# YukunXia/SuperPoint-Stereo-Visual-Odometry

Measured on AMD Instinct MI355X. Metric: stereo frames/sec (1241x376 KITTI), higher is better.
Workload: dtype f32

## Files before the change

superpoint-stereo-visual-odometry_amd/csrc/conv_wino4.hip.h:

```cpp
#pragma once
#include <hip/hip_runtime.h>
#include <stdint.h>
#include <type_traits>
#include <vector>
#include "conv_mfma.hip.h"

#ifndef WINO4_LEAD
#define WINO4_LEAD 6
#endif
#ifndef WINO4_PRIO
#define WINO4_PRIO 1
#endif
#ifndef WINO4_H1_STEPS
#define WINO4_H1_STEPS 6
#endif
#ifndef WINO4_H1_START
#define WINO4_H1_START 3
#endif
#ifndef WINO4_H1_STRIDE
#define WINO4_H1_STRIDE 5
#endif
#ifndef WINO4_H2_START
#define WINO4_H2_START 4
#endif
#ifndef WINO4_H2_STRIDE
#define WINO4_H2_STRIDE 8
#endif
#ifndef WINO4_ABL
#define WINO4_ABL 0
#endif

#ifndef SPVO_STATIC_BANDS
#define SPVO_STATIC_BANDS 1
#endif

namespace spvo {

template <int TB>
struct Wino4TileT {
  static constexpr int CK = 4, TH = 8 * TB, TW = 32, LW = TW + 8, LH = TH + 2, NT = 16 * TB, NTH = 256 * TB;
  static constexpr int IN_FLOATS = CK * LH * LW;
  static constexpr int U_FLOATS = 36 * CK * CO_TILE;
  static constexpr int V_FLOATS = 10 * TB * 64 * 4;
  static constexpr int RAW_OFF = 0, U_OFF = 2 * IN_FLOATS, V_OFF = U_OFF + 2 * U_FLOATS;
  static constexpr int LDS_BYTES = (V_OFF + 2 * V_FLOATS) * 4 + 16;
};
using Wino4Tile = Wino4TileT<2>;

inline std::vector<float> pack_conv_weights_wino4(const float *w, const float *bias, int cout, int cin) {
  constexpr int CK = Wino4Tile::CK;
  const int co_tiles = (cout + CO_TILE - 1) / CO_TILE, nch = cin / CK;
  std::vector<float> out((size_t)co_tiles * nch * Wino4Tile::U_FLOATS + (size_t)co_tiles * CO_TILE, 0.f);
  static const double G[6][3] = {{0.25, 0, 0}, {-1.0 / 6, -1.0 / 6, -1.0 / 6}, {-1.0 / 6, 1.0 / 6, -1.0 / 6},
                                 {1.0 / 24, 1.0 / 12, 1.0 / 6}, {1.0 / 24, -1.0 / 12, 1.0 / 6}, {0, 0, 1}};
  for (int ct = 0; ct < co_tiles; ++ct)
    for (int o = 0; o < CO_TILE; ++o) {
      const int co = ct * CO_TILE + o;
      if (co >= cout) continue;
      out[(size_t)co_tiles * nch * Wino4Tile::U_FLOATS + co] = bias[co];
      for (int ci = 0; ci < cin; ++ci) {
        const float *g = w + ((size_t)co * cin + ci) * 9;
        double t[6][3];
        for (int a = 0; a < 6; ++a)
          for (int k = 0; k < 3; ++k) t[a][k] = G[a][0] * g[0 * 3 + k] + G[a][1] * g[1 * 3 + k] + G[a][2] * g[2 * 3 + k];
        float *slab = out.data() + ((size_t)ct * nch + ci / CK) * Wino4Tile::U_FLOATS;
        const int lane = 16 * (ci % CK) + (o & 15), cq = o >> 4;
        for (int a = 0; a < 6; ++a)
          for (int b = 0; b < 6; ++b) {
            const int pos = 18 * (b / 3) + 3 * a + b % 3;
            slab[(((pos >> 2) * 4 + cq) * 64 + lane) * 4 + (pos & 3)] = (float)(t[a][0] * G[b][0] + t[a][1] * G[b][1] + t[a][2] * G[b][2]);
          }
      }
    }
  return out;
}

__device__ __forceinline__ void wino4_in6(const float x0, const float x1, const float x2, const float x3, const float x4, const float x5, float (&o)[6]) {
  const float e = fmaf(-4.f, x2, x4), od = fmaf(-4.f, x1, x3), e2 = x4 - x2, o2 = x3 - x1;
  o[0] = fmaf(4.f, x0, fmaf(-5.f, x2, x4));
  o[1] = e + od;
  o[2] = e - od;
  o[3] = fmaf(2.f, o2, e2);
  o[4] = fmaf(-2.f, o2, e2);
  o[5] = fmaf(4.f, x1, fmaf(-5.f, x3, x5));
}
__device__ __forceinline__ void wino4_out4(const float m0, const float m1, const float m2, const float m3, const float m4, const float m5, float (&y)[4]) {
  const float a = m1 + m2, b = m1 - m2, c = m3 + m4, d = m3 - m4;
  y[0] = (m0 + a) + c;
  y[1] = fmaf(2.f, d, b);
  y[2] = fmaf(4.f, c, a);
  y[3] = fmaf(8.f, d, b) + m5;
}

typedef float wino4_f32x2 __attribute__((ext_vector_type(2)));
__device__ __forceinline__ void wino4_out4(const wino4_f32x2 m0, const wino4_f32x2 m1, const wino4_f32x2 m2, const wino4_f32x2 m3, const wino4_f32x2 m4,
                                           const wino4_f32x2 m5, wino4_f32x2 (&y)[4]) {
  const wino4_f32x2 a = m1 + m2, b = m1 - m2, c = m3 + m4, d = m3 - m4;
  y[0] = (m0 + a) + c;
  y[1] = __builtin_elementwise_fma(wino4_f32x2{2.f, 2.f}, d, b);
  y[2] = __builtin_elementwise_fma(wino4_f32x2{4.f, 4.f}, c, a);
  y[3] = __builtin_elementwise_fma(wino4_f32x2{8.f, 8.f}, d, b) + m5;
}

template <bool POOL, bool RELU, int TAG = 0, int TB = 2>
__global__ __launch_bounds__(256 * TB, TB) void conv_wino4_kernel(const ConvArgs a) {
  using T = Wino4TileT<TB>;
  constexpr int CK = T::CK, LW = T::LW, LH = T::LH, LW4 = LW / 4, NTH = T::NTH;
  constexpr int IN_V4 = T::IN_FLOATS / 4;
  constexpr int U_V4 = T::U_FLOATS / 4;
  constexpr int NIT_U = (U_V4 + NTH - 1) / NTH;
  typedef float f32x2 __attribute__((ext_vector_type(2)));
  typedef float f32x4v __attribute__((ext_vector_type(4)));

  extern __shared__ __attribute__((aligned(16))) float smem[];

  const int tid = threadIdx.x;
  const int lane = tid & 63;
  const int c16 = lane & 15, g4 = lane >> 4;
  const int wave = __builtin_amdgcn_readfirstlane(tid >> 6);
  const int cq = wave & 3, tb = wave >> 2;
  const size_t in_plane = (size_t)a.in_hp * a.in_wp;
  const size_t out_plane = (size_t)a.out_hp * a.out_wp;
  const int n_tiles = a.tiles_x * a.tiles_y * a.co_tiles * a.batch;

  struct TileRef { const float *in_base, *w_base; int x0, y0, ct, img; };
  auto decode = [&](int id) {
    TileRef t;
    const int tx = id % a.tiles_x;
    id /= a.tiles_x;
    const int ty = id % a.tiles_y;
    id /= a.tiles_y;
    t.ct = id % a.co_tiles;
    t.img = id / a.co_tiles;
    t.x0 = tx * T::TW;
    t.y0 = ty * T::TH;
    t.in_base = a.in + ((size_t)t.img * a.in_ctot + a.in_coff) * in_plane + (size_t)(t.y0 + PADY - 1) * a.in_wp + (t.x0 + PADX - 4);
    t.w_base = a.wpack + (size_t)t.ct * a.n_chunks * T::U_FLOATS;
    return t;
  };

  auto raw_piece_off = [&](int idx) {
    idx = min(idx, IN_V4 - 1);
    const int ci = idx / (LH * LW4);
    const int rem = idx - ci * (LH * LW4);
    const int r = rem / LW4;
    const int q = rem - r * LW4;
    return 4u * (unsigned)(ci * (int)in_plane + r * a.in_wp + q * 4);
  };
  constexpr int R0 = NTH - 256;
  const unsigned roff0 = raw_piece_off(tid), roff1 = raw_piece_off(NTH + (tid - R0));
  const bool raw2 = tid >= R0 && NTH + (tid - R0) < IN_V4;
  auto issue_raw = [&](const TileRef &t, int chunk, float *buf) {
    const char *inb = reinterpret_cast<const char *>(t.in_base + (size_t)chunk * CK * in_plane);
    glds16(reinterpret_cast<const float *>(inb + roff0), buf + (wave * 64) * 4);
    if (raw2) glds16(reinterpret_cast<const float *>(inb + roff1), buf + (NTH + (wave - R0 / 64) * 64) * 4);
  };
  const unsigned uoff = 16u * (unsigned)tid;
  auto issue_u = [&](const TileRef &t, int chunk, float *buf) {
    const char *wb = reinterpret_cast<const char *>(t.w_base + (size_t)chunk * T::U_FLOATS);
#pragma unroll
    for (int it = 0; it < NIT_U; ++it)
      if (it < NIT_U - 1 || tid < U_V4 - (NIT_U - 1) * NTH) glds16(reinterpret_cast<const float *>(wb + (uoff + 16u * NTH * it)), buf + (it * NTH + wave * 64) * 4);
  };

  const int x_ci = TB == 2 ? (wave & 3) : 2 * (wave & 1) + ((lane >> 4) & 1), x_tile = TB == 2 ? (lane & 31) : (lane & 15), x_h = lane >> 5;
  const int x_trow = x_tile >> 3, x_tcol = x_tile & 7;
  const int raw_off = x_ci * (LH * LW) + (4 * x_trow + 3 * x_h) * LW + 4 * x_tcol + 3;
  const int v_off = x_h * (1280 * TB) + (x_tile >> 4) * 256 + (16 * x_ci + (x_tile & 15)) * 4;
  float xr[3][6];
  f32x4v xa[3];
  float xs0[3], xs1[3];
  auto xf_step = [&](const float *raw, float *vb, int st) {
    if (st < 3) {
      const float *d = raw + raw_off + st * LW;
      xs0[st] = d[0];
      xa[st] = *reinterpret_cast<const f32x4v *>(d + 1);
      xs1[st] = d[5];
    } else if (st < 6) {
      const int r = st - 3;
      wino4_in6(xs0[r], xa[r][0], xa[r][1], xa[r][2], xa[r][3], xs1[r], xr[r]);
    } else if (st == 6) {
#pragma unroll
      for (int r = 0; r < 3; ++r)
#pragma unroll
        for (int c = 0; c < 3; ++c) {
          typedef unsigned u32x2s __attribute__((ext_vector_type(2)));
          const u32x2s sw = __builtin_amdgcn_permlane32_swap(__float_as_uint(xr[r][c]), __float_as_uint(xr[r][c + 3]), false, false);
          xr[r][c] = __uint_as_float(sw[0]);
          xr[r][c + 3] = __uint_as_float(sw[1]);
        }
    } else {
      const int c = st - 7;
      float o[6];
      wino4_in6(xr[0][c], xr[1][c], xr[2][c], xr[0][c + 3], xr[1][c + 3], xr[2][c + 3], o);
#pragma unroll
      for (int i = 0; i < 6; ++i) vb[v_off + ((3 * i + c) >> 2) * (256 * TB) + ((3 * i + c) & 3)] = o[i];
    }
  };

  const int a_lane = cq * 64 + lane;
  const int b_lane = tb * 64 + lane;

  const int band = blockIdx.x & 7;
  auto wgs_before = [&](int b) { return min(b, (int)gridDim.x & 7) + b * ((int)gridDim.x >> 3); };
  auto band_lo = [&](int b) { return (int)((long)n_tiles * wgs_before(b) / (int)gridDim.x); };
  auto band_hi = [&](int b) { return band_lo(b + 1); };
  auto band_wgs = [&](int b) { return wgs_before(b + 1) - wgs_before(b); };
  auto steal = [&]() {
    for (int k = 1; k < 8; ++k) {
      const int b = (band + k) & 7;
      if (band_lo(b) + band_wgs(b) >= band_hi(b)) continue;
      const int v = band_lo(b) + band_wgs(b) + atomicAdd(a.sched + b, 1);
      if (v < band_hi(b)) return v;
    }
    return n_tiles;
  };
  auto all_done = [&]() {
    if (a.sched && tid == 0 && atomicAdd(a.sched + 8, 1) == (int)gridDim.x - 1)
      for (int k = 0; k < 9; ++k) a.sched[k] = 0;
  };
  int *const sched_slot = reinterpret_cast<int *>(smem + (T::LDS_BYTES - 16) / 4);
  int tile_id = SPVO_STATIC_BANDS ? wgs_before(band) + ((int)blockIdx.x >> 3) : (int)blockIdx.x;
  if (a.sched) {
    tile_id = band_lo(band) + (blockIdx.x >> 3);
    if (tile_id >= band_hi(band)) {
      if (tid == 0) *sched_slot = steal();
      __syncthreads();
      tile_id = *sched_slot;
      __syncthreads();
    }
  }
  if (tile_id >= n_tiles) {
    all_done();
    return;
  }
  TileRef cur = decode(tile_id);

  int nxt_id = tile_id + gridDim.x;
  int dyn_fetch = 0;
  struct Cursor { TileRef t; int chunk, id; };
  auto advance = [&](Cursor &q) {
    if (++q.chunk == a.n_chunks) {
      asm volatile("" ::: "memory");
      q.chunk = 0;
      q.id = a.sched ? nxt_id : q.id + (int)gridDim.x;
      if (q.id < n_tiles) q.t = decode(q.id);
    }
  };
  Cursor cu{cur, 0, tile_id};
  issue_raw(cu.t, 0, smem + T::RAW_OFF);
  issue_u(cu.t, 0, smem + T::U_OFF);
  advance(cu);
  if (cu.id < n_tiles) issue_raw(cu.t, cu.chunk, smem + T::RAW_OFF + T::IN_FLOATS);
  Cursor cr = cu;
  advance(cr);
  asm volatile("s_waitcnt vmcnt(0)\n\ts_barrier" ::: "memory");
  if (wave < 2 * TB) {
#pragma unroll
    for (int st = 0; st < 10; ++st) xf_step(smem + T::RAW_OFF, smem + T::V_OFF, st);
  } else {
#pragma unroll
    for (int st = 0; st < WINO4_H1_STEPS; ++st) xf_step(smem + T::RAW_OFF + T::IN_FLOATS, smem + T::V_OFF + T::V_FLOATS, st);
  }
  asm volatile("s_waitcnt lgkmcnt(0)\n\ts_barrier" ::: "memory");
  if (cr.id < n_tiles) issue_raw(cr.t, cr.chunk, smem + T::RAW_OFF);
  advance(cr);

#ifdef WINO_STAMPS
  unsigned long long st_dma = 0, st_bar = 0, st_mfma = 0, st_epi = 0, st_items = 0, st_post = 0, st_bar_xf = 0, st_mfma_xf = 0;
  const unsigned long long st_t0 = __builtin_amdgcn_s_memtime(), st_r0 = __builtin_amdgcn_s_memrealtime();
  int st_c = 0;
#endif
  int k = 0;
  bool drained = false;
  constexpr unsigned OOB = 0xFFFFFFFFu;

  while (tile_id < n_tiles) {
    if (a.sched) {
      if (tid == 0) dyn_fetch = band_lo(band) + band_wgs(band) + atomicAdd(a.sched + band, 1);
    } else {
      nxt_id = tile_id + gridDim.x;
    }

    f32x4v acc[36];
    auto item = [&](auto first_tag, bool publish) {
      constexpr bool FIRST = decltype(first_tag)::value;
      const bool XF = __builtin_amdgcn_readfirstlane((wave >> TB) == (k & 1) ? 1 : 0) != 0;
#ifdef WINO_STAMPS
      const unsigned long long ts0 = __builtin_amdgcn_s_memtime();
#endif
      if (!drained) asm volatile("s_waitcnt vmcnt(0)" ::: "memory");
      drained = false;
#ifdef WINO_STAMPS
      const unsigned long long ts1 = __builtin_amdgcn_s_memtime();
#endif
      if (publish && tid == 0) *sched_slot = dyn_fetch < band_hi(band) ? dyn_fetch : n_tiles;
      asm volatile("s_waitcnt lgkmcnt(0)\n\ts_barrier" ::: "memory");
      if (publish) nxt_id = __builtin_amdgcn_readfirstlane(*sched_slot);
#ifdef WINO_STAMPS
      const unsigned long long ts2 = __builtin_amdgcn_s_memtime();
      st_dma += ts1 - ts0; st_bar += ts2 - ts1;
      if (st_c == 1) st_post += ts1 - ts0;
      if (XF) st_bar_xf += ts2 - ts1;
#endif
      const float *ub = smem + T::U_OFF + (k & 1) * T::U_FLOATS;
      const float *vb = smem + T::V_OFF + (k & 1) * T::V_FLOATS;
      float *u_next = smem + T::U_OFF + ((k + 1) & 1) * T::U_FLOATS;
      const float *raw_next2 = smem + T::RAW_OFF + (k & 1) * T::IN_FLOATS;
      float *raw_next3 = smem + T::RAW_OFF + ((k + 1) & 1) * T::IN_FLOATS;
      float *v_next = smem + T::V_OFF + ((k + 1) & 1) * T::V_FLOATS;
      const f32x4v *ub4 = reinterpret_cast<const f32x4v *>(ub) + a_lane;
      const f32x4v *vb4 = reinterpret_cast<const f32x4v *>(vb) + b_lane;
      constexpr int LEAD = WINO4_LEAD;
      f32x4v av[9], bv[10];
      auto b_piece = [](int p) { return 5 * (p / 18) + ((p % 18) >> 2); };
#pragma unroll
      for (int p = 0; p < ((WINO4_ABL & 8) ? 36 : LEAD); ++p) {
        if ((WINO4_ABL & 8) && k > 0) break;
        if ((p & 3) == 0) av[p >> 2] = ub4[(p >> 2) * 256];
        if (p == 0 || b_piece(p) != b_piece(p - 1)) bv[b_piece(p)] = vb4[b_piece(p) * (64 * TB)];
      }
#pragma unroll
      for (int p = 0; p < 36; ++p) {
        const int ph = p / 18, pq = p % 18, pos = 6 * (pq / 3) + 3 * ph + pq % 3;
        const float a_op = av[p >> 2][p & 3], b_op = bv[b_piece(p)][pq & 3];
#if WINO4_PRIO
#if WINO4_PRIO == 1
        if (p == 0) asm volatile("s_setprio 3");
        if (p == 9) asm volatile("s_setprio 2");
        if (p == 18) asm volatile("s_setprio 1");
        if (p == 27) asm volatile("s_setprio 0");
#elif WINO4_PRIO == 2
        if (p == 0) asm volatile("s_setprio 3");
        if (tb == 0) { if (p == 6) asm volatile("s_setprio 2"); if (p == 15) asm volatile("s_setprio 1"); if (p == 24) asm volatile("s_setprio 0"); }
        else { if (p == 12) asm volatile("s_setprio 2"); if (p == 24) asm volatile("s_setprio 1"); }
#elif WINO4_PRIO == 3
        if (p == 0) asm volatile("s_setprio 1");
        if (p == 18) asm volatile("s_setprio 0");
#elif WINO4_PRIO == 4
        if (tb == 0) { if (p == 0) asm volatile("s_setprio 2"); if (p == 12) asm volatile("s_setprio 1"); if (p == 24) asm volatile("s_setprio 0"); }
        else { if (p == 0) asm volatile("s_setprio 3"); if (p == 12) asm volatile("s_setprio 2"); if (p == 24) asm volatile("s_setprio 1"); }
#endif
#endif
        if (FIRST) acc[pos] = __builtin_amdgcn_mfma_f32_16x16x4f32(a_op, b_op, f32x4v{0.f, 0.f, 0.f, 0.f}, 0, 0, 0);
        else acc[pos] = __builtin_amdgcn_mfma_f32_16x16x4f32(a_op, b_op, acc[pos], 0, 0, 0);
        __builtin_amdgcn_sched_barrier(0);
        if (!(WINO4_ABL & 2) && p == 1 && cu.id < n_tiles) issue_u(cu.t, cu.chunk, u_next);
        if (!(WINO4_ABL & 4) && p == 4 && cr.id < n_tiles) issue_raw(cr.t, cr.chunk, raw_next3);
        const int q = p + LEAD;
        if (!(WINO4_ABL & 8) && q < 36) {
          if ((q & 3) == 0) av[q >> 2] = ub4[(q >> 2) * 256];
          if (b_piece(q) != b_piece(q - 1)) bv[b_piece(q)] = vb4[b_piece(q) * (64 * TB)];
        }
        if (!(WINO4_ABL & 1) && XF && p >= WINO4_H1_START && p < WINO4_H1_START + WINO4_H1_STEPS * WINO4_H1_STRIDE && (p - WINO4_H1_START) % WINO4_H1_STRIDE == 0)
          xf_step(raw_next2, v_next, (p - WINO4_H1_START) / WINO4_H1_STRIDE);
        if (!(WINO4_ABL & 1) && !XF && p >= WINO4_H2_START && p < WINO4_H2_START + (10 - WINO4_H1_STEPS) * WINO4_H2_STRIDE && (p - WINO4_H2_START) % WINO4_H2_STRIDE == 0)
          xf_step(raw_next2, v_next, WINO4_H1_STEPS + (p - WINO4_H2_START) / WINO4_H2_STRIDE);
        __builtin_amdgcn_sched_barrier(0);
      }
      advance(cu);
      advance(cr);
      ++k;
#ifdef WINO_STAMPS
      { const unsigned long long dt = __builtin_amdgcn_s_memtime() - ts2; st_mfma += dt; if (XF) st_mfma_xf += dt; }
      ++st_items; ++st_c;
#endif
    };
#ifdef WINO_STAMPS
    st_c = 0;
#endif
    item(std::true_type{}, false);
    for (int c = 1; c < a.n_chunks; ++c) item(std::false_type{}, a.sched != nullptr && c == 1);

#ifdef WINO_STAMPS
    const unsigned long long te0 = __builtin_amdgcn_s_memtime();
#endif
    asm volatile("s_waitcnt vmcnt(0)" ::: "memory");
    drained = true;

    const int co0 = cur.ct * CO_TILE + cq * 16 + 4 * g4;
    float *co_base = a.out + (((size_t)cur.img * a.out_ctot + a.out_coff) + (size_t)cur.ct * CO_TILE + cq * 16) * out_plane;
    const __amdgpu_buffer_rsrc_t rsrc = __builtin_amdgcn_make_buffer_rsrc(co_base, 0, 0x7FFFFFFF, 0x00020000);
    const int oplane = (int)out_plane;
    const int kmax = a.cout - co0;
    const float *bias_p = a.wpack + (size_t)a.co_tiles * a.n_chunks * T::U_FLOATS + min(co0, a.cout - 1);
    const int trow = 2 * tb + (c16 >> 3), tcol = c16 & 7;
    auto relu = [](float v) { return RELU ? __builtin_amdgcn_fmed3f(v, 0.f, __builtin_inff()) : v; };
    const int oy = cur.y0 + 4 * trow, ox = cur.x0 + 4 * tcol;
#pragma unroll
    for (int rp = 0; rp < 2; ++rp) {
      typedef wino4_f32x2 f32x2;
      const f32x2 bias_v = {bias_p[2 * rp < kmax ? 2 * rp : 0], bias_p[2 * rp + 1 < kmax ? 2 * rp + 1 : 0]};
      auto pr = [&](int p) { return f32x2{acc[p][2 * rp], acc[p][2 * rp + 1]}; };
      f32x2 z[6][4];
#pragma unroll
      for (int j = 0; j < 6; ++j) wino4_out4(pr(0 + j), pr(6 + j), pr(12 + j), pr(18 + j), pr(24 + j), pr(30 + j), z[j]);
      f32x2 y2[4][4];
#pragma unroll
      for (int i = 0; i < 4; ++i) {
        wino4_out4(z[0][i], z[1][i], z[2][i], z[3][i], z[4][i], z[5][i], y2[i]);
#pragma unroll
        for (int jj = 0; jj < 4; ++jj) y2[i][jj] += bias_v;
      }
#pragma unroll
      for (int e = 0; e < 2; ++e) {
      const int r = 2 * rp + e;
      float y[4][4];
#pragma unroll
      for (int i = 0; i < 4; ++i)
#pragma unroll
        for (int jj = 0; jj < 4; ++jj) y[i][jj] = relu(y2[i][jj][e]);
      const bool ch_ok = r < kmax;
      if constexpr (POOL) {
        typedef unsigned u32x2 __attribute__((ext_vector_type(2)));
        const int ow = a.W >> 1;
#pragma unroll
        for (int pi = 0; pi < 2; ++pi) {
          float pv[2];
#pragma unroll
          for (int pj = 0; pj < 2; ++pj)
            pv[pj] = fmaxf(fmaxf(y[2 * pi][2 * pj], y[2 * pi][2 * pj + 1]), fmaxf(y[2 * pi + 1][2 * pj], y[2 * pi + 1][2 * pj + 1]));
          const int py = (oy >> 1) + pi, px = ox >> 1;
          const unsigned vo = (ch_ok && py < (a.H >> 1) && px < ow) ? 4u * (unsigned)(4 * g4 * oplane + (py + PADY) * a.out_wp + (px + PADX)) : OOB;
          const u32x2 v = {__float_as_uint(pv[0]), __float_as_uint(px + 1 < ow ? pv[1] : 0.f)};
          __builtin_amdgcn_raw_buffer_store_b64(v, rsrc, (WINO4_ABL & 16) ? OOB : vo, r * oplane * 4, 0);
        }
      } else {
        typedef unsigned u32x4 __attribute__((ext_vector_type(4)));
#pragma unroll
        for (int i = 0; i < 4; ++i) {
          const int yy = oy + i;
          const unsigned vo = (ch_ok && yy < a.H && ox < a.W) ? 4u * (unsigned)(4 * g4 * oplane + (yy + PADY) * a.out_wp + (ox + PADX)) : OOB;
          const u32x4 v = {__float_as_uint(y[i][0]), __float_as_uint(ox + 1 < a.W ? y[i][1] : 0.f), __float_as_uint(ox + 2 < a.W ? y[i][2] : 0.f),
                           __float_as_uint(ox + 3 < a.W ? y[i][3] : 0.f)};
          __builtin_amdgcn_raw_buffer_store_b128(v, rsrc, (WINO4_ABL & 16) ? OOB : vo, r * oplane * 4, 0);
        }
      }
      }
      __builtin_amdgcn_sched_barrier(0);
    }
#ifdef WINO_STAMPS
    st_epi += __builtin_amdgcn_s_memtime() - te0;
#endif
    tile_id = nxt_id;
    if (tile_id < n_tiles) cur = decode(tile_id);
  }
  all_done();
#ifdef WINO_STAMPS
  if (lane == 0 && a.stamps) {
    unsigned long long *o = a.stamps + 8 * (blockIdx.x * (4 * TB) + wave);
    o[0] = st_dma; o[1] = st_bar; o[2] = st_mfma; o[3] = st_epi; o[4] = st_items;
    o[5] = __builtin_amdgcn_s_memtime() - st_t0; o[6] = __builtin_amdgcn_s_memrealtime() - st_r0; o[7] = st_post;
#ifdef WINO_STAMPS_ROLES
    o[0] = st_mfma_xf; o[7] = st_bar_xf;
#endif
  }
#endif
}

}
```

Baseline: 1517.

## Load Winograd weight tiles directly into registers instead of staging through LDS

By default the transformed weight (U) pieces now go from global memory straight into registers with buffer loads, running several pieces ahead of the MFMA loop, instead of being DMA-staged into double-buffered LDS. This frees LDS space and removes the LDS reads for the A operand. The raw-input loads become buffer_load_lds, and the per-chunk wait relaxes to vmcnt(8) so outstanding weight prefetches do not block. It adds register pressure and exposes the MFMA loop to global memory latency, and the partial vmcnt count is fragile if the load ordering changes.

```diff
diff --git a/superpoint-stereo-visual-odometry_amd/csrc/conv_wino4.hip.h b/superpoint-stereo-visual-odometry_amd/csrc/conv_wino4.hip.h
--- a/superpoint-stereo-visual-odometry_amd/csrc/conv_wino4.hip.h
+++ b/superpoint-stereo-visual-odometry_amd/csrc/conv_wino4.hip.h
@@ -30,6 +30,14 @@
 #define WINO4_ABL 0
 #endif
 
+#ifndef WINO4_U_LDS
+#define WINO4_U_LDS 0
+#endif
+
+#ifndef WINO4_A_AHEAD
+#define WINO4_A_AHEAD 5
+#endif
+
 #ifndef SPVO_STATIC_BANDS
 #define SPVO_STATIC_BANDS 1
 #endif
@@ -42,7 +50,7 @@
   static constexpr int IN_FLOATS = CK * LH * LW;
   static constexpr int U_FLOATS = 36 * CK * CO_TILE;
   static constexpr int V_FLOATS = 10 * TB * 64 * 4;
-  static constexpr int RAW_OFF = 0, U_OFF = 2 * IN_FLOATS, V_OFF = U_OFF + 2 * U_FLOATS;
+  static constexpr int RAW_OFF = 0, U_OFF = 2 * IN_FLOATS, V_OFF = U_OFF + (WINO4_U_LDS ? 2 * U_FLOATS : 0);
   static constexpr int LDS_BYTES = (V_OFF + 2 * V_FLOATS) * 4 + 16;
 };
 using Wino4Tile = Wino4TileT<2>;
@@ -151,10 +159,18 @@
   const unsigned roff0 = raw_piece_off(tid), roff1 = raw_piece_off(NTH + (tid - R0));
   const bool raw2 = tid >= R0 && NTH + (tid - R0) < IN_V4;
   auto issue_raw = [&](const TileRef &t, int chunk, float *buf) {
+#if WINO4_U_LDS
     const char *inb = reinterpret_cast<const char *>(t.in_base + (size_t)chunk * CK * in_plane);
     glds16(reinterpret_cast<const float *>(inb + roff0), buf + (wave * 64) * 4);
     if (raw2) glds16(reinterpret_cast<const float *>(inb + roff1), buf + (NTH + (wave - R0 / 64) * 64) * 4);
-  };
+#else
+    const __amdgpu_buffer_rsrc_t rr = __builtin_amdgcn_make_buffer_rsrc(const_cast<float *>(t.in_base + (size_t)chunk * CK * in_plane), 0, 0x7FFFFFFF, 0x00020000);
+    typedef __attribute__((address_space(3))) void *lds_ptr;
+    __builtin_amdgcn_raw_ptr_buffer_load_lds(rr, (lds_ptr)(buf + (wave * 64) * 4), 16, (int)roff0, 0, 0, 0);
+    if (raw2) __builtin_amdgcn_raw_ptr_buffer_load_lds(rr, (lds_ptr)(buf + (NTH + (wave - R0 / 64) * 64) * 4), 16, (int)roff1, 0, 0, 0);
+#endif
+  };
+#if WINO4_U_LDS
   const unsigned uoff = 16u * (unsigned)tid;
   auto issue_u = [&](const TileRef &t, int chunk, float *buf) {
     const char *wb = reinterpret_cast<const char *>(t.w_base + (size_t)chunk * T::U_FLOATS);
@@ -162,6 +178,15 @@
     for (int it = 0; it < NIT_U; ++it)
       if (it < NIT_U - 1 || tid < U_V4 - (NIT_U - 1) * NTH) glds16(reinterpret_cast<const float *>(wb + (uoff + 16u * NTH * it)), buf + (it * NTH + wave * 64) * 4);
   };
+#else
+  const unsigned aoff = 16u * (unsigned)(cq * 64 + lane);
+  auto a_piece = [&](const TileRef &t, int chunk, int j) {
+    typedef unsigned u32x4 __attribute__((ext_vector_type(4)));
+    const __amdgpu_buffer_rsrc_t wr = __builtin_amdgcn_make_buffer_rsrc(const_cast<float *>(t.w_base), 0, 0x7FFFFFFF, 0x00020000);
+    const u32x4 v = __builtin_amdgcn_raw_buffer_load_b128(wr, aoff, 4 * (chunk * T::U_FLOATS + 1024 * j), 0);
+    return __builtin_bit_cast(f32x4v, v);
+  };
+#endif
 
   const int x_ci = TB == 2 ? (wave & 3) : 2 * (wave & 1) + ((lane >> 4) & 1), x_tile = TB == 2 ? (lane & 31) : (lane & 15), x_h = lane >> 5;
   const int x_trow = x_tile >> 3, x_tcol = x_tile & 7;
@@ -198,7 +223,9 @@
     }
   };
 
+#if WINO4_U_LDS
   const int a_lane = cq * 64 + lane;
+#endif
   const int b_lane = tb * 64 + lane;
 
   const int band = blockIdx.x & 7;
@@ -226,7 +253,7 @@
     if (tile_id >= band_hi(band)) {
       if (tid == 0) *sched_slot = steal();
       __syncthreads();
-      tile_id = *sched_slot;
+      tile_id = __builtin_amdgcn_readfirstlane(*sched_slot);
       __syncthreads();
     }
   }
@@ -249,7 +276,13 @@
   };
   Cursor cu{cur, 0, tile_id};
   issue_raw(cu.t, 0, smem + T::RAW_OFF);
+#if WINO4_U_LDS
   issue_u(cu.t, 0, smem + T::U_OFF);
+#else
+  f32x4v av[9];
+#pragma unroll
+  for (int j = 0; j < WINO4_A_AHEAD; ++j) av[j] = a_piece(cu.t, 0, j);
+#endif
   advance(cu);
   if (cu.id < n_tiles) issue_raw(cu.t, cu.chunk, smem + T::RAW_OFF + T::IN_FLOATS);
   Cursor cr = cu;
@@ -265,6 +298,9 @@
   asm volatile("s_waitcnt lgkmcnt(0)\n\ts_barrier" ::: "memory");
   if (cr.id < n_tiles) issue_raw(cr.t, cr.chunk, smem + T::RAW_OFF);
   advance(cr);
+#if !WINO4_U_LDS
+  asm volatile("s_waitcnt vmcnt(0)" ::: "memory");
+#endif
 
 #ifdef WINO_STAMPS
   unsigned long long st_dma = 0, st_bar = 0, st_mfma = 0, st_epi = 0, st_items = 0, st_post = 0, st_bar_xf = 0, st_mfma_xf = 0;
@@ -272,7 +308,12 @@
   int st_c = 0;
 #endif
   int k = 0;
-  bool drained = false;
+  bool drained = !WINO4_U_LDS;
+#if WINO4_U_LDS || (WINO4_ABL & 2)
+#define WINO4_WAIT_RAW "s_waitcnt vmcnt(0)"
+#else
+#define WINO4_WAIT_RAW "s_waitcnt vmcnt(8)"
+#endif
   constexpr unsigned OOB = 0xFFFFFFFFu;
 
   while (tile_id < n_tiles) {
@@ -283,13 +324,13 @@
     }
 
     f32x4v acc[36];
-    auto item = [&](auto first_tag, bool publish) {
+    auto item = [&](auto first_tag, bool publish, int chunk) {
       constexpr bool FIRST = decltype(first_tag)::value;
       const bool XF = __builtin_amdgcn_readfirstlane((wave >> TB) == (k & 1) ? 1 : 0) != 0;
 #ifdef WINO_STAMPS
       const unsigned long long ts0 = __builtin_amdgcn_s_memtime();
 #endif
-      if (!drained) asm volatile("s_waitcnt vmcnt(0)" ::: "memory");
+      if (!drained) asm volatile(WINO4_WAIT_RAW ::: "memory");
       drained = false;
 #ifdef WINO_STAMPS
       const unsigned long long ts1 = __builtin_amdgcn_s_memtime();
@@ -303,21 +344,28 @@
       if (st_c == 1) st_post += ts1 - ts0;
       if (XF) st_bar_xf += ts2 - ts1;
 #endif
+#if WINO4_U_LDS
       const float *ub = smem + T::U_OFF + (k & 1) * T::U_FLOATS;
+      float *u_next = smem + T::U_OFF + ((k + 1) & 1) * T::U_FLOATS;
+      const f32x4v *ub4 = reinterpret_cast<const f32x4v *>(ub) + a_lane;
+#endif
       const float *vb = smem + T::V_OFF + (k & 1) * T::V_FLOATS;
-      float *u_next = smem + T::U_OFF + ((k + 1) & 1) * T::U_FLOATS;
       const float *raw_next2 = smem + T::RAW_OFF + (k & 1) * T::IN_FLOATS;
       float *raw_next3 = smem + T::RAW_OFF + ((k + 1) & 1) * T::IN_FLOATS;
       float *v_next = smem + T::V_OFF + ((k + 1) & 1) * T::V_FLOATS;
-      const f32x4v *ub4 = reinterpret_cast<const f32x4v *>(ub) + a_lane;
       const f32x4v *vb4 = reinterpret_cast<const f32x4v *>(vb) + b_lane;
       constexpr int LEAD = WINO4_LEAD;
-      f32x4v av[9], bv[10];
+#if WINO4_U_LDS
+      f32x4v av[9];
+#endif
+      f32x4v bv[10];
       auto b_piece = [](int p) { return 5 * (p / 18) + ((p % 18) >> 2); };
 #pragma unroll
       for (int p = 0; p < ((WINO4_ABL & 8) ? 36 : LEAD); ++p) {
         if ((WINO4_ABL & 8) && k > 0) break;
+#if WINO4_U_LDS
         if ((p & 3) == 0) av[p >> 2] = ub4[(p >> 2) * 256];
+#endif
         if (p == 0 || b_piece(p) != b_piece(p - 1)) bv[b_piece(p)] = vb4[b_piece(p) * (64 * TB)];
       }
 #pragma unroll
@@ -345,11 +393,21 @@
         if (FIRST) acc[pos] = __builtin_amdgcn_mfma_f32_16x16x4f32(a_op, b_op, f32x4v{0.f, 0.f, 0.f, 0.f}, 0, 0, 0);
         else acc[pos] = __builtin_amdgcn_mfma_f32_16x16x4f32(a_op, b_op, acc[pos], 0, 0, 0);
         __builtin_amdgcn_sched_barrier(0);
+#if WINO4_U_LDS
         if (!(WINO4_ABL & 2) && p == 1 && cu.id < n_tiles) issue_u(cu.t, cu.chunk, u_next);
+#else
+        if (!(WINO4_ABL & 2) && (p & 3) == 3) {
+          const int g = (p >> 2) + WINO4_A_AHEAD;
+          if (g < 9) av[g] = a_piece(cur, chunk, g);
+          else av[g - 9] = a_piece(cu.t, cu.chunk, g - 9);
+        }
+#endif
         if (!(WINO4_ABL & 4) && p == 4 && cr.id < n_tiles) issue_raw(cr.t, cr.chunk, raw_next3);
         const int q = p + LEAD;
         if (!(WINO4_ABL & 8) && q < 36) {
+#if WINO4_U_LDS
           if ((q & 3) == 0) av[q >> 2] = ub4[(q >> 2) * 256];
+#endif
           if (b_piece(q) != b_piece(q - 1)) bv[b_piece(q)] = vb4[b_piece(q) * (64 * TB)];
         }
         if (!(WINO4_ABL & 1) && XF && p >= WINO4_H1_START && p < WINO4_H1_START + WINO4_H1_STEPS * WINO4_H1_STRIDE && (p - WINO4_H1_START) % WINO4_H1_STRIDE == 0)
@@ -369,13 +427,13 @@
 #ifdef WINO_STAMPS
     st_c = 0;
 #endif
-    item(std::true_type{}, false);
-    for (int c = 1; c < a.n_chunks; ++c) item(std::false_type{}, a.sched != nullptr && c == 1);
+    item(std::true_type{}, false, 0);
+    for (int c = 1; c < a.n_chunks; ++c) item(std::false_type{}, a.sched != nullptr && c == 1, c);
 
 #ifdef WINO_STAMPS
     const unsigned long long te0 = __builtin_amdgcn_s_memtime();
 #endif
-    asm volatile("s_waitcnt vmcnt(0)" ::: "memory");
+    asm volatile(WINO4_WAIT_RAW ::: "memory");
     drained = true;
 
     const int co0 = cur.ct * CO_TILE + cq * 16 + 4 * g4;
```

Result: no change. 1531 (median of 6 runs) (+0.9%).
